# niclasborlin/dbat

Hardware: AMD Instinct MI355X
Metric: LM iterations/sec (higher is better)
Workload: dtype f64

## Files before the change

### dbat_amd/_hip.py

```python
from __future__ import annotations

import ctypes as C
import os
import sys

import numpy as np

_HERE = os.path.dirname(os.path.abspath(__file__))
LIB_PATH = os.path.join(_HERE, 'libdbat_hip.so')
if os.environ.get('DBAT_AMD_LIB') == 'prof':
    LIB_PATH = os.path.join(_HERE, 'libdbat_hip_prof.so')
elif os.environ.get('DBAT_AMD_LIB', '').endswith('.so'):
    LIB_PATH = os.environ['DBAT_AMD_LIB']
if LIB_PATH != os.path.join(_HERE, 'libdbat_hip.so'):
    sys.stderr.write('[dbat_amd] DBAT_AMD_LIB: loading %s instead of the product library\n' % LIB_PATH)

ABI_VERSION = 5
DAMP = {'none': 0, 'gm': 0, 'gna': 1, 'lm': 2, 'lmp': 3}

OK, EINVAL, EUNSUPPORTED, EDEVICE, ENOMEM = 0, -101, -102, -103, -104


class DbatHipUnavailable(RuntimeError):
    pass
# ... 138 lines not shown
    'dbat_hip_ray_angles': (C.c_int, [_H, _dp, _dp, _dp, _ip, _ip]),
    'dbat_hip_debug_ray_angles_host': (C.c_int, [C.POINTER(Problem), _dp, _dp]),
    'dbat_hip_default_robust_options': (C.c_int, [C.c_int32, C.POINTER(RobustOptions)]),
    'dbat_hip_robust_weights': (C.c_int, [_H, _dp, C.POINTER(RobustOptions), _dp, _dp, _dp]),
    'dbat_hip_set_obs_weights': (C.c_int, [_H, _dp]),
    'dbat_hip_solve_robust': (C.c_int, [_H, C.POINTER(Options), C.POINTER(RobustOptions), _dp, C.POINTER(Result),
                                        _dp, _dp, _dp, _dp, C.POINTER(RobustResult), _dp]),
}
DEBUG_SYMBOLS = {
    'dbat_hip_debug_plan_digest': (C.c_int, [C.POINTER(Problem), C.POINTER(C.c_uint64), C.c_int32, C.c_char_p, C.c_int32]),
    'dbat_hip_debug_heavy_plan_selftest': (C.c_int, [C.POINTER(Problem), _dp]),
    'dbat_hip_debug_batch_stats': (C.c_int, [C.POINTER(Problem), C.POINTER(C.c_int64)]),
    'dbat_hip_debug_model_eval_host': (C.c_int, [C.c_int32, C.c_int32, C.c_int32, _dp, _dp, C.c_double,
                                                 _dp, _dp, _dp, _dp, _dp, _dp]),
    'dbat_hip_debug_ray_angles_ms': (C.c_int, [_H, _dp, C.POINTER(C.c_int64)]),
}

_lib = None


def load():
    global _lib
    if _lib is not None:
        return _lib
    if not os.path.exists(LIB_PATH):
        raise DbatHipUnavailable(
            '%s not built: run `python -c "import __graft_entry__ as g; g.build()"` or '
            '`make -C dbat_amd/csrc` (needs hipcc).  There is no CPU fallback.' % LIB_PATH)
    try:
        try:
# ... 407 lines not shown
    def set_x(self, x):
        x = np.ascontiguousarray(x, float)
        check(self.lib.dbat_hip_set_x(self.h, dptr(x)))

    def bench_step(self, lam=0.0, scale=False):
        ms = np.zeros(16)
        check(self.lib.dbat_hip_bench_step(self.h, float(lam), int(bool(scale)), dptr(ms)))
        return ms

    def chol_stats(self):
        a = (C.c_int64 * 6)()
        check(self.lib.dbat_hip_chol_stats(self.h, a))
        keys = ('order_padded', 'tile_tasks', 'tile_products', 'tile_rows', 'nested_dissection', 'dataflow')
        return dict(zip(keys, [int(v) for v in a]))

    def info(self):
        a = (C.c_int64 * 24)()
        check(self.lib.dbat_hip_info(self.h, a))
        keys = ('NS', 'n_batches', 'max_k', 'n_obs_shard', 'n_pts_shard', 'BT', 'ncolmax', 'n_tiles',
                'domain_sharding', 'reduced_doubles_per_factorisation', 'vector_doubles_per_linearisation',
                'n_top_cams', 'factor_tile_rows', 'tasks_domain', 'tasks_top', 'tile_kernel_mfma',
                'heavy_tasks', 'heavy_mfma', 'heavy_row_groups', 'heavy_scratch_bytes', 'heavy_points', 'heavy_obs',
                'heavy_ksteps_per_task', 'heavy_algorithmic_flops')
        return dict(zip(keys, [int(v) for v in a]))


def structure_key(s, device=0, shard_rank=0, shard_count=1, _problem=None):
    prob, keep = _problem if _problem is not None else problem_from_struct(s, device, shard_rank, shard_count)
    k = (C.c_uint64 * 2)()
    check(load().dbat_hip_structure_key(C.byref(prob), k))
# ... 178 lines not shown
```

### dbat_amd/csrc/dbat_core.hip

```cpp
#include <hip/hip_runtime.h>
#include <rocblas/rocblas.h>
#include <rocsolver/rocsolver.h>
#include <rccl/rccl.h>

#include <chrono>
#include <cmath>
#include <cstdio>
#include <cstdlib>
#include <memory>
#include <string>
#include <thread>
#include <type_traits>
#include <utility>
#include <atomic>
#include <vector>

#include "../../include/dbat_hip.h"
#include "chol_df.hpp"
#include "kernels.hpp"
#include "sig.hpp"
#include "heavy.hpp"
#include "plan.hpp"
#include "resect.hpp"
#include "robust.hpp"
// ... 104 lines not shown
    enum class TileRoute { none, sig, tile3, tile2 } route = TileRoute::none;
    DevBuf<int64_t> o_row, batch_start, x2z, giant_start, cm_chunk_start;
    DevBuf<int32_t> cm_pt, cm_chunk_cam, tile_order;
    DevBuf<double> cm_uv, cm_w;
    int64_t n_cm_chunks = 0, n_cm_chunks_all = 0;
    DevBuf<double> giant_W;
    int64_t ngiant = 0;
    bool use_heavy = false;
    HeavyDev hv{};
    DevBuf<int32_t> hv_obs_dst, hv_pt_io0, hv_io_dst, hv_io_pt, hv_pt_y, hv_grp_nb, hv_grp_row, hv_task, hv_ops;
    DevBuf<uint8_t> hv_obs_ld, hv_obs_ioloc, hv_io_ld;
    DevBuf<double> hv_Z;
    int giant_threads = 256;
    DevBuf<CamRec> cams, cams_f;
    bool cams_at_lin = false;

    const char *env_df_trace = nullptr;
    DevBuf<unsigned> gctr;
    DevBuf<double> gpart, rpart;
    DevBuf<double> z, zt, dz, zlin, vtmp, vtmp2, xbuf;
    DevBuf<double> red;
    DevBuf<double> jn2c, dscale, rhs, Vinv, gp, jn2p, partial, scal;
    DevBuf<int> info;
    DevBuf<double> linv, ldiag;
    DataflowChol dfchol;
    DataflowChol dfchol_ip;
    bool use_perm = true;
    bool mg_subtree = false;
    DevBuf<uint8_t> piv_have;
    bool chol_in_place = false;
// ... 205 lines not shown
        lds_cov = ((size_t)P.BT * P.ncolmax * 3 + (size_t)P.BT * 6) * sizeof(double);
        tile2_pc = TILE2_PC;
        static_assert(Plan::PMAX == 256 / 2, "k_build_tile2 / k_build_tile3 lay out NPROD / 2 points per batch");
        lds_tile2 = ((size_t)TILE2_NBUF * 3 * tile2_pc * TILE_LD + (size_t)2 * Plan::PMAX * 9 + (size_t)Plan::PMAX * 15 + TILE_LD) * sizeof(double);
        lds_tile3 = ((size_t)TILE3_NBUF * 3 * TILE3_PC * TILE_LD + (size_t)2 * Plan::PMAX * 9 + (size_t)2 * Plan::PMAX * 9 + TILE_LD) * sizeof(double);
        use_tile2 = P.BT == 256 && P.ncolmax <= 15;
        if (ntiles <= 0) route = TileRoute::none;
        else if (use_sig) route = TileRoute::sig;
        else if (use_tile2 && !P.with_io && tile_ncx == 6) route = TileRoute::tile3;
        else if (use_tile2 && (tile_ncx == 14 || tile_ncx == 15)) route = TileRoute::tile2;
        else throw DeviceError{"internal: tiles without a tile kernel"};
        partial.alloc((size_t)4 * std::max<int64_t>(std::max<int64_t>(std::max<int64_t>(nb + ntiles + ngiant + (int64_t)P.sg_chunk.size() / 8, n_cm_chunks_all), 2048), 1));
        HIPCHK(hipMemcpy(z.p, P.z0.data(), P.NZ * 8, hipMemcpyHostToDevice));
        HIPCHK(hipMemset(dz.p, 0, P.NZ * 8));
        HIPCHK(hipMemset(zt.p, 0, P.NZ * 8));
        precompute_image_side();
        HIPCHK(hipDeviceSynchronize());
        lapi("work arrays, image side");
    }

    void precompute_image_side() {
        uv_pre = !P.with_io;
        d.o_uv_raw = o_uv.p; d.uv_pre = uv_pre ? 1 : 0;
        if (!uv_pre || nobs == 0) return;
        prep_cams(z.p, cams_f.p);
        if (!o_rhs.p) o_rhs.alloc((size_t)2 * nobs);
        with_value<2, 3, 4, 5>(P.model, [&](auto M) {
            launch<k_uv_to_rhs<M>>(dim3((unsigned)cdiv(nobs, 256)), dim3(256), 0, d.nK, d.nP, cams_f.p, nobs, o_cam.p, o_uv.p, o_rhs.p);
            if (n_cm_chunks_all > 0) launch<k_uv_to_rhs_cm<M>>(dim3((unsigned)n_cm_chunks_all), dim3(256), 0, d.nK, d.nP, cams_f.p, cm_chunk_cam.p, cm_chunk_start.p, cm_uv.p);
            if (use_sig && sg_nchunks > 0) launch<k_uv_to_rhs_sig<M>>(dim3((unsigned)sg_nchunks), dim3(64), 0, d.nK, d.nP, cams_f.p, sg_chunk.p, sg_gcam.p, sg_uv.p);
// ... 6 lines not shown
        HIPCHK(hipMemcpyAsync(z.p, P.z0.data(), P.NZ * 8, hipMemcpyHostToDevice, stream));
        HIPCHK(hipMemcpyAsync(io_fixed.p, P.io_fixed.data(), P.io_fixed.size() * 8, hipMemcpyHostToDevice, stream));
        if (d.any_prior) {
            HIPCHK(hipMemcpyAsync(z_prw.p, P.z_prw.data(), P.NZ * 8, hipMemcpyHostToDevice, stream));
            HIPCHK(hipMemcpyAsync(z_prv.p, P.z_prv.data(), P.NZ * 8, hipMemcpyHostToDevice, stream));
        }
        HIPCHK(hipStreamSynchronize(stream));
        if (uv_pre && io_changed && nobs > 0) {
            HIPCHK(hipMemcpy(cm_uv.p, P.cm_uv.data(), P.cm_uv.size() * 8, hipMemcpyHostToDevice));
            if (use_sig && sg_nchunks > 0) HIPCHK(hipMemcpy(sg_uv.p, P.sg_uv.data(), P.sg_uv.size() * 8, hipMemcpyHostToDevice));
            d.o_uv = o_uv.p;
            precompute_image_side();
            HIPCHK(hipStreamSynchronize(stream));
        }
        cams_at_lin = false; have_lin = false; s_valid = false; pend_build = false; lin_pending = false;
        lambda_lin = 0; scale_lin = 0; f_lin = 0; trace_jtj = 0; near_singular = false; chol_in_place = false; replicate_next = false;
        n_res_evals = n_lin = n_solves = n_trace_only = 0;
    }

    static int env_grid_obs() { return std::min(std::max(1, env_int("DBAT_HIP_GRID_OBS", 1536)), 1 << 20); }

    int64_t tile_kernel_mfma() const {
        if (route == TileRoute::none) return 0;
        int64_t n = 0;
        if (route == TileRoute::sig) {
            for (int64_t t = 0; t < ntiles; ++t) {
                const int nio = tile_ncx > 6 ? P.tile_io_start[t + 1] - P.tile_io_start[t] : 0;
                for (int64_t q = P.sg_tile_chunk0[t]; q < P.sg_tile_chunk0[t + 1]; ++q) {
                    const int npts = P.sg_chunk[8 * q + 1], k = P.sg_chunk[8 * q + 2];
                    const int ppr = std::min(SIG_PPR, 64 / std::max(k, 1)), rbk = (6 * k + nio + 1 + 15) >> 4;
// ... 92 lines not shown
        do_allreduce(zgather.p, P.NZ);
        return zgather.p;
    }
    void read_scal(double *host, int n) {
        if (n <= 32) {
            HIPCHK(hipMemcpyAsync(hpin, scal.p, n * sizeof(double), hipMemcpyDeviceToHost, stream));
            sync();
            memcpy(host, hpin, n * sizeof(double));
            return;
        }
        HIPCHK(hipMemcpyAsync(host, scal.p, n * sizeof(double), hipMemcpyDeviceToHost, stream));
        sync();
    }
    void prep_cams(const double *zz, CamRec *into = nullptr) {
        if (!into) { into = cams.p; cams_at_lin = false; }
        launch<k_cam_prep>(dim3((unsigned)cdiv(P.nc, 64)), dim3(64), 0, d, zz, into);
    }
    void x_to_z(const double *x_host, double *z_dev) {
        HIPCHK(hipMemcpyAsync(z_dev, P.z0.data(), P.NZ * 8, hipMemcpyHostToDevice, stream));
        if (P.n) {
            HIPCHK(hipMemcpyAsync(xbuf.p, x_host, P.n * 8, hipMemcpyHostToDevice, stream));
            launch<k_scatter_x>(dim3((unsigned)cdiv(P.n, 256)), dim3(256), 0, P.n, x2z.p, xbuf.p, z_dev);
        }
    }
    void z_to_x(const double *z_dev, double *x_host) {
        if (!P.n) return;
        stage(4);
        z_dev = gathered(z_dev);
        launch<k_gather_x>(dim3((unsigned)cdiv(P.n, 256)), dim3(256), 0, P.n, x2z.p, z_dev, xbuf.p);
        HIPCHK(hipMemcpyAsync(x_host, xbuf.p, P.n * 8, hipMemcpyDeviceToHost, stream));
        sync();
    }

// ... 25 lines not shown
        if (!P.n || nt <= 0) return std::max(nt, 0);
        HIPCHK(hipMemcpyAsync(host, trace_dev.p, (size_t)P.n * nt * 8, hipMemcpyDeviceToHost, stream));
        HIPCHK(hipStreamSynchronize(stream));
        for (int k = 0; k < nt; ++k)
            if (!trace_have[k]) std::fill(host + (size_t)P.n * k, host + (size_t)P.n * (k + 1), NAN);
        if ((size_t)P.n * trace_cap * 8 > ((size_t)256 << 20)) {
            DevBuf<double> old;
            std::swap(old.p, trace_dev.p);
            trace_cap = 0;
        }
        return nt;
    }

    double eval_f_step(const double *x, double alpha, const double *pdir, double *out) {
        stage(3);
        if ((int64_t)cdiv(P.NZ, 256) < P.nc) { axpby(1.0, x, alpha, pdir, out); return eval_f(out, nullptr, nullptr); }
        launch<k_axpby_cams>(dim3((unsigned)cdiv(P.NZ, 256)), dim3(256), 0, d, 1.0, x, alpha, pdir, out, cams_f.p);
        return eval_f(out, nullptr, nullptr, true);
    }
    double eval_f(const double *zz, double *r_w_out, double *r_unw_out, bool cams_ready = false) {
        stage(3);
        if (!cams_ready) prep_cams(zz, cams_f.p);
        mark(6);
        const bool res_tail = n_cm_chunks_all > 0 && n_cm_chunks_all <= 512 && !d.any_prior && !multi() && !r_w_out && !r_unw_out;
        with_value<2, 3, 4, 5>(P.model, [&](auto M) {
            with_value<false, true>(uv_pre, [&](auto PRE) {
                if (n_cm_chunks_all > 0)
                    launch<k_residual_cm<M, PRE>>(dim3((unsigned)n_cm_chunks_all), dim3(256), 0, d, zz, cams_f.p, cm_pt.p, cm_uv.p, pw ? cm_w.p : (const double *)nullptr,
                                                  cm_chunk_cam.p, cm_chunk_start.p, partial.p, res_tail ? gctr.p + 1 : (unsigned *)nullptr, scal.p, hpin, res_tail ? ++mb_seq : 0ull);
                mark(7);
                if (r_w_out || r_unw_out) launch<k_residual<M, PRE>>(dim3(grid_obs), dim3(256), 0, d, zz, cams_f.p, rpart.p, r_w_out, r_unw_out);
            });
        });
// ... 167 lines not shown
            for (int i = 0; i < 8; ++i) fprintf(stderr, " %s=%.2f", nm[i], h[i] * 0.01 / (double)std::max<int64_t>(ntiles, 1));
            fprintf(stderr, "\n");
            memset(h, 0, sizeof(h));
            HIPCHK(hipMemcpyToSymbol(HIP_SYMBOL(g_tile2_prof), h, sizeof(h)));
        } else if ((d.ablate & 32) && use_tile2) {
            unsigned long long h[16];
            HIPCHK(hipStreamSynchronize(stream));
            HIPCHK(hipMemcpyFromSymbol(h, HIP_SYMBOL(g_tile2_prof), sizeof(h)));
            static const char *nm[12] = {"stage(wait freed)", "P1", "pbarrier", "P2", "P3", "drain", "cons wait full", "cons zero+free", "tail/flush", "loop head", "cons product", "cons wait done"};
            fprintf(stderr, "[tile2 prof, us per tile avg over %d tiles]", (int)ntiles);
            for (int i = 0; i < 12; ++i) fprintf(stderr, " %s=%.2f", nm[i], h[i] * 0.01 / (double)std::max<int64_t>(ntiles, 1));
            fprintf(stderr, "\n");
            memset(h, 0, sizeof(h));
            HIPCHK(hipMemcpyToSymbol(HIP_SYMBOL(g_tile2_prof), h, sizeof(h)));
        }
        launch<k_build_tail>(dim3(grid_zs), dim3(1024), 0, d, zz, partial.p, npart, jn2p.p, gpart.p, gctr.p + 2, red_scal,
                zz != zlin.p ? zlin.p : (double *)nullptr);
    }
    bool pend_build = false;
    double pend_lambda = 0;
    int pend_scale = 0;
    void request_build(double lambda, int scale) {
        pend_build = true; pend_lambda = lambda; pend_scale = scale;
        lambda_lin = lambda; scale_lin = scale;
    }
    void ensure_build() {
        if (!pend_build) return;
        build(z.p, pend_lambda, pend_scale, true);
    }
    void settle_lin_point() {
        if (!pend_build) return;
        copy(zlin.p, z.p);
        cams_at_lin = false; s_valid = false; have_lin = true;
    }
    void allreduce_vectors() {
        if (!multi()) return;
        do_allreduce(g_c, 2 * P.NS + 8);
    }
    void trace_only_pass(const double *zz) {
        stage(0);
        prep_cams(zz);
        if (n_cm_chunks_all > 0) {
            with_value<2, 3, 4, 5>(P.model, [&](auto M) { with_value<6, 14, 15, MAXCOL>(tile_ncx, [&](auto NCX) {
                launch<k_trace_cm<M, NCX>>(dim3((unsigned)n_cm_chunks_all), dim3(256), 0, d, zz, cams.p, cm_pt.p, cm_uv.p, pw ? cm_w.p : (const double *)nullptr,
                                           cm_chunk_cam.p, cm_chunk_start.p, partial.p);
            }); });
        }
// ... 37 lines not shown
        launch<k_finish>(dim3((unsigned)cdiv(P.NS, 256)), dim3(256), 0, d, zz, lambda, scale, S, g_c, g_red, diagU, jn2c.p, dscale.p,
                gpart.p, gctr.p + 3, (const double *)red_scal, scal.p, hpin, mg_subtree && multi() ? (const uint8_t *)z_mine.p : (const uint8_t *)nullptr,
                ride ? info.p : (int *)nullptr, ride ? df_ctl : (int *)nullptr, ride ? df_q : (unsigned long long *)nullptr, ride ? df_nq : 0);
        if (ride) dfchol.reset_done = true;
        if (scale)
            launch<k_envelope_op>(dim3((unsigned)P.NS), dim3(256), 0, S, ldS, (int)P.NS, env_tail0, col_bend.p, (const double *)dscale.p, (double *)nullptr,
                                  (unsigned long long *)nullptr);
    }

    int factor_solve_enqueue() {
        if (mg_subtree && !multi())
            throw UsageError{"this handle is one of several shards: attach a communicator (dbat_hip_comm_init) or an all-reduce "
                             "callback (dbat_hip_set_allreduce) before linearising or solving"};
        stage(1);
        mark(2);
        if (use_perm && !chol_in_place && mg_subtree && multi()) {
            dfchol.solve_domain(stream, S, ldS, linv.p, info.p, ldiag.p);
            mark(8);
            do_allreduce(dfchol.top_tiles(), dfchol.top_tiles_count());
            mark(9);
            dfchol.solve_top(stream, ldS, rhs.p, linv.p, info.p, ldiag.p, dscale.p, dz.p);
        } else if (use_perm && !chol_in_place) dfchol.solve(stream, S, ldS, rhs.p, linv.p, info.p, ldiag.p, dscale.p, dz.p);
        else dfchol_ip.solve(stream, S, ldS, rhs.p, linv.p, info.p, ldiag.p, dscale.p, dz.p);
        HIPCHK(hipGetLastError());
        if (env_df_trace) (use_perm && !chol_in_place ? dfchol : dfchol_ip).dump_trace(stream, env_df_trace);
        mark(3);
        ++n_solves;
        return 0;
    }
    void backsub_enqueue() {
        stage(2);
        mark(4);
        const bool sig_bs = use_sig && P.sg_backsub_ok;
        const int64_t b_first = sig_bs ? P.nb_tiled : 0;
        const int64_t n_sig_wg = sig_bs ? cdiv(sg_nchunks, 4) : 0;
        if (n_sig_wg > 0) {
            with_value<2, 3, 4, 5>(P.model, [&](auto M) { with_value<6, 14>(tile_ncx, [&](auto NCX) {
                launch<k_backsub_sig<M, NCX>>(dim3((unsigned)n_sig_wg), dim3(256), 0, d, zlin.p, cams.p, Vinv.p, gp.p, dz.p, partial.p + 2 * (nb + ngiant), sg_chunk.p,
                                              (int)sg_nchunks, sg_gcam.p, sg_uv.p, pw ? sg_w.p : (const double *)nullptr);
            }); });
        }
        if (nb > b_first) {
            with_value<2, 3, 4, 5>(P.model, [&](auto M) { with_value<6, 14, 15, MAXCOL>(tile_ncx, [&](auto NCX) {
                launch<k_backsub<M, NCX>>(dim3((unsigned)(nb - b_first)), dim3(P.BT), lds_back, d, zlin.p, cams.p, Vinv.p, gp.p, dz.p, partial.p, (int)b_first);
            }); });
        }
        if (ngiant > 0) {
            with_value<2, 3, 4, 5>(P.model, [&](auto M) { with_value<false, true>(P.with_io, [&](auto IO) {
                launch<k_backsub_giant<M, IO>>(dim3((unsigned)ngiant), dim3(giant_threads), 0, d, zlin.p, cams.p, Vinv.p, gp.p, dz.p, partial.p + 2 * nb);
            }); });
        }
        mark(5);
        launch<k_prior_jv>(dim3(grid_zs), dim3(1024), 0, d, zlin.p, dz.p, g_c, gp.p, gpart.p, gctr.p + 4,
                (const double *)(partial.p + 2 * b_first), nb - b_first + ngiant + n_sig_wg, (const double *)ldiag.p, pivmm.p,
                (const int *)info.p, scal.p, multi() ? (double *)nullptr : hpin, ++mb_seq,
                mg_subtree && multi() ? (const uint8_t *)piv_have.p : (const uint8_t *)nullptr);
    }
    bool near_singular = false;
    const bool pivot_stats = env_on("DBAT_HIP_PIVOT_STATS");
    double rcond_est = 0.0;
    int chol_info = 0;
    double piv_last[4] = {0, 0, 0, 0};
    bool solve(double &JpJp, double &rJp, double &pp) {
        ensure_build();
        if (!s_valid) build(zlin.p, lambda_lin, scale_lin);
        s_valid = false;
        factor_solve_enqueue();
// ... 391 lines not shown
                                         (const double *)o_w_base.p, o_w.p, (const int32_t *)(use_sig ? sg_map.p : nullptr), sg_w.p,
                                         (const int32_t *)cm_map.p, cm_w.p);
        s_valid = false;
    }
    void robust_omega_ip(double *host) {
        if (!robust_on) { std::fill(host, host + P.no, 1.0); return; }
        DevBuf<double> t;
        t.alloc((size_t)std::max<int64_t>(P.no, 1));
        HIPCHK(hipMemsetAsync(t.p, 0, (size_t)P.no * sizeof(double), stream));
        if (nobs > 0) launch<k_scatter_rows1>(dim3(robust_grid()), dim3(256), 0, nobs, (const int64_t *)o_row.p, (const double *)omega.p, t.p);
        if (multi()) do_allreduce(t.p, P.no);
        HIPCHK(hipMemcpyAsync(host, t.p, (size_t)P.no * sizeof(double), hipMemcpyDeviceToHost, stream));
        HIPCHK(hipStreamSynchronize(stream));
    }
    void jtimes(const double *v, double &JvJv, double &rJv, double &vv) {
        if (!cams_at_lin) { prep_cams(zlin.p); cams_at_lin = true; }
        with_value<2, 3, 4, 5>(P.model, [&](auto M) { with_value<6, 14, 15, MAXCOL>(tile_ncx, [&](auto NCX) {
            launch<k_jtimes<M, NCX>>(dim3(grid_obs), dim3(256), 0, d, zlin.p, cams.p, v, partial.p);
        }); });
        launch<k_prior_jv>(dim3(grid_zs), dim3(1024), 0, d, zlin.p, v, g_c, gp.p, gpart.p, gctr.p + 4,
                (const double *)partial.p, (int64_t)grid_obs, (const double *)nullptr, pivmm.p, (const int *)info.p, scal.p, (double *)nullptr, 0ull, (const uint8_t *)nullptr);
        do_allreduce(scal.p, 8);
        double h[8];
        read_scal(h, 8);
        JvJv = h[0] + h[4]; rJv = h[1] + h[5]; vv = h[6];
    }
    double dot_owned(const double *a, const double *b) {
        launch<k_dot>(dim3(grid_z), dim3(256), 0, P.NZ, z_mine.p, a, b, partial.p);
        launch<k_sum_partials<1>>(dim3(1), dim3(1024), 0, partial.p, (int64_t)grid_z, scal.p, 0);
        do_allreduce(scal.p, 1);
        double s;
        read_scal(&s, 1);
        return s;
    }
    void axpby(double a, const double *x, double b, const double *y2, double *y) {
        launch<k_axpby>(dim3((unsigned)cdiv(P.NZ, 256)), dim3(256), 0, P.NZ, a, x, b, y2, y);
    }
    void gradient(double *g) {
        launch<k_gradient>(dim3((unsigned)cdiv(P.NZ, 256)), dim3(256), 0, d, g_c, gp.p, g);
    }
    void colnorm2(double *out) {
        launch<k_jn2>(dim3((unsigned)cdiv(P.NZ, 256)), dim3(256), 0, d, jn2c.p, jn2p.p, out);
    }
    void jac_blocks(const double *zz, double *a, double *b, double *cc) {
        with_value<2, 3, 4, 5>(P.model, [&](auto M) { launch<k_jac_blocks<M>>(dim3((unsigned)cdiv(nobs, 256)), dim3(256), 0, d, zz, cams.p, a, b, cc); });
    }
    void copy(double *dst, const double *src) { HIPCHK(hipMemcpyAsync(dst, src, P.NZ * 8, hipMemcpyDeviceToDevice, stream)); }
    void accept_trial() { std::swap(z.p, zt.p); }
};


struct LoopOut {
    std::vector<double> res, damp, aux;
    int code = 0, iters = 0;
    double f_final = 0;
};

static void export_residuals(Core &c, const double *zdev, double *r_unw, double *r_wgt, double *f);
static void jtimes_rows(Core &c, const double *v_dev, double *Jv);

static void keep_Jp(Core &c, const dbat_hip_options &o, const double *p_dev, std::vector<double> &Jp) {
    if (!o.term_fun) return;
    Jp.resize((size_t)c.P.m);
// ... 1219 lines not shown
    if (!h || !st) { g_err = "null argument"; return DBAT_HIP_EINVAL; }
    const Core &c = *h->core;
    const DataflowChol &f = c.use_perm ? c.dfchol : c.dfchol_ip;
    st[0] = f.n; st[1] = f.ntasks; st[2] = f.n_products; st[3] = f.nT; st[4] = c.use_perm ? 1 : 0; st[5] = 1;
    return DBAT_HIP_OK;
}

int dbat_hip_build_kernel_name(const dbat_hip_handle *h, char *buf, int32_t buf_len) {
    if (!h || !buf || buf_len < 2) { g_err = "null argument"; return DBAT_HIP_EINVAL; }
    const Core &c = *h->core;
    using R = Core::TileRoute;
    const char *nm = c.route == R::sig ? "k_build_sig" : c.route == R::tile3 ? "k_build_tile3" : c.route == R::tile2 ? "k_build_tile2"
                   : c.use_heavy ? "k_heavy_z + k_heavy_syrk" : "k_build";
    snprintf(buf, (size_t)buf_len, "%s", nm);
    return DBAT_HIP_OK;
}

int dbat_hip_info(const dbat_hip_handle *h, int64_t *info) {
    if (!h || !info) { g_err = "null argument"; return DBAT_HIP_EINVAL; }
    const Core &c = *h->core;
    info[0] = c.P.NS; info[1] = c.nb; info[2] = c.P.max_k; info[3] = c.nobs;
    info[4] = c.P.pt_hi - c.P.pt_lo; info[5] = c.P.BT; info[6] = c.P.ncolmax; info[7] = c.ntiles;
    info[8] = c.mg_subtree ? 1 : 0;
    info[9] = c.mg_subtree ? c.dfchol.top_tiles_count() : (c.P.nranks > 1 ? c.pk_s_count : 0);
    info[10] = c.P.nranks > 1 ? (c.mg_subtree ? 2 * c.P.NS + 8 : 3 * c.P.NS + 8) : 0;
    info[11] = c.mg_subtree ? c.P.nd.n_top_cams : 0;
    info[12] = c.use_perm ? c.dfchol.nT : 0;
    info[13] = c.mg_subtree ? c.dfchol.ntasks : 0; info[14] = c.mg_subtree ? c.dfchol.ntasksB : 0;
    info[15] = c.tile_kernel_mfma();
    for (int i = 16; i < 24; ++i) info[i] = 0;
// ... 187 lines not shown
```

### dbat_amd/csrc/env.hpp

```cpp
#pragma once
#include <cstdlib>
#include <cstring>
#include <string>

extern char **environ;

namespace dbat {

#ifdef DBAT_HIP_PROFILING
constexpr bool kProfilingBuild = true;
#else
constexpr bool kProfilingBuild = false;
#endif

struct EnvSwitch { const char *name; bool measurement; const char *what; const char *values = nullptr; };
static const EnvSwitch kEnvSwitches[] = {
    {"DBAT_HIP_SIG", false, "0: signature kernels off, 2: on wherever a chunk's rows fit (default: by group length)", "0|1|2"},
    {"DBAT_HIP_SIG_IOS_OFF", false, "self-calibration: IO rows by LDS atomics in every tile"},
    {"DBAT_HIP_CMAX", false, "cameras per tile (0: column-list kernel only)"},
    {"DBAT_HIP_BT", false, "observations per batch (128 | 256)", "128|256"},
    {"DBAT_HIP_TILE_BMIN", false, "fewest batches a tile may be capped at (default 2)"},
    {"DBAT_HIP_HEAVY", false, "0: heavy / giant points by the column-list kernels (pair terms by global atomics) instead of the matrix-core path", "0|1"},
    {"DBAT_HIP_HEAVY_KS", false, "heavy / giant points: k-steps per task of k_heavy_syrk at most (default: by the amount of work, 12 ... 96)"},
    {"DBAT_HIP_GIANT_THREADS", false, "threads of the giant-point kernels (64 | 128 | 256)", "64|128|256"},
// ... 1 lines not shown
    {"DBAT_HIP_ND_OFF", false, "no nested dissection"},
    {"DBAT_HIP_ND_LEAF", false, "leaf size of the dissection"},
    {"DBAT_HIP_ND_PAD_ALL", false, "every block of the dissection on a tile boundary"},
    {"DBAT_HIP_ND_JOIN_SMALL", false, "separators up to that many rows join their child's last tile"},
    {"DBAT_HIP_DF_SPLIT", false, "factorisation: helper tasks for sums longer than this many products (default 96)"},
    {"DBAT_HIP_DF_CHUNK", false, "factorisation: products per helper task (default 32)"},
    {"DBAT_HIP_DF_CHAIN", false, "factorisation: 0 = diagonal tiles as ordinary tasks (no chain role), 1 = chain role whatever the pattern", "0|1"},
    {"DBAT_HIP_DF_CHAIN_WG", false, "factorisation: workgroups of the chain role at most (default 32)"},
    {"DBAT_HIP_DF_L2", false, "factorisation: 1 = finished tiles of the compact layout are read through the L2", "0|1"},
    {"DBAT_HIP_COV_DENSE", false, "posterior covariance: the dense inverse of the reduced system (rocsolver_dpotri) instead of the selected inversion"},
    {"DBAT_HIP_SPRANK_OFF", false, "structural rank from the counting conditions only"},
    {"DBAT_HIP_PLAN_THREADS", false, "threads of the host plan (default: hardware concurrency, at most 32)"},
    {"DBAT_HIP_PLAN_GRAIN", false, "elements per thread below which a pass of the host plan is not split (tests: 1)"},
    {"DBAT_HIP_PLAN_STATS", false, "1: print layout statistics, 2: also the wall time of every section of the plan"},
    {"DBAT_HIP_PIVOT_STATS", false, "print the pivot extremes and the rcond estimate of every solve"},
    {"DBAT_HIP_ABLATE", true, "k_build_sig / tile kernels: switch phases off (results are wrong), phase clocks"},
    {"DBAT_HIP_DF_TRACE", true, "per-task clocks of the factorisation, written to this file"},
    {"DBAT_HIP_DF_TRACE_POTF2", true, "with DF_TRACE: clocks inside the chain role's factorisations as well"},
    {"DBAT_HIP_DF_ABLATE", true, "factorisation: operand tiles of the products not fetched (1: L(i,j), 2: both, 3: and no flag looks) -- timing only, wrong results", "0|1|2|3"},
    {"DBAT_HIP_DF_ORDER", true, "one of the candidate task orders instead of the simulated best"},
    {"DBAT_HIP_DF_GRID", true, "workgroups of the factorisation"},
    {"DBAT_HIP_GRID_OBS", true, "launch size of the observation-parallel kernels"},
};

inline const char *env_get(const char *name) {
    for (const EnvSwitch &e : kEnvSwitches)
        if (!strcmp(e.name, name)) return (e.measurement && !kProfilingBuild) ? nullptr : getenv(name);
    return nullptr;
}
inline int env_int(const char *name, int dflt) { const char *e = env_get(name); return e ? atoi(e) : dflt; }
// ... 27 lines not shown
```

### dbat_amd/csrc/kernels.hpp

```cpp
#pragma once
#include <hip/hip_runtime.h>

#include "model.hpp"

namespace dbat {

struct DevProblem {
    int nc, np, nIOrows, nK, nP, nIOu, ncolmax, BT;
    int64_t NS, NZ, nobs, nb;
    int64_t ldS;
    const int32_t *cam_ncol, *cam_col, *cam_iorow;
    const uint32_t *cam_eo_est;
    const int32_t *io_src;
    const double *io_fixed;
    const double *px;
    const double *cam_w;
    const uint8_t *z_est, *z_mine;
    const double *z_prw, *z_prv;
    const int32_t *o_cam, *o_pt;
    const double *o_uv;
    const double *o_uv_raw;
    int uv_pre;
    const double *o_w;
    const uint32_t *o_seg;
// ... 2729 lines not shown
        out[0] = acc[3]; out[1] = acc[4]; out[4] = acc[0]; out[5] = acc[1]; out[6] = acc[2];
        out[7] = info && __hip_atomic_load(info, __ATOMIC_RELAXED, __HIP_MEMORY_SCOPE_AGENT) != 0 ? 1.0 : 0.0;
        out[2] = 0.0; out[3] = 0.0;
        if (mailbox) {
            mailbox[0] = acc[3]; mailbox[1] = acc[4]; mailbox[4] = acc[0]; mailbox[5] = acc[1]; mailbox[6] = acc[2];
            for (int q = 0; q < 4; ++q)
                mailbox[40 + q] = __longlong_as_double((long long)__hip_atomic_load(pivmm + q, __ATOMIC_RELAXED, __HIP_MEMORY_SCOPE_AGENT));
            const int hi = __hip_atomic_load(info, __ATOMIC_RELAXED, __HIP_MEMORY_SCOPE_AGENT);
            long long w = hi;
            mailbox[44] = __longlong_as_double(w);
            mailbox_done(mailbox, seq);
        }
    }
}

__global__ __launch_bounds__(256) void k_dot(int64_t n, const uint8_t *__restrict__ mine,
                                             const double *__restrict__ a, const double *__restrict__ b ,
                                             double *__restrict__ partial) {
    __shared__ double sh[8];
    double acc[1] = {0};
    const int64_t stride = (int64_t)gridDim.x * blockDim.x;
    for (int64_t i = (int64_t)blockIdx.x * blockDim.x + threadIdx.x; i < n; i += stride)
        if (!mine || mine[i]) acc[0] += a[i] * (b ? b[i] : 1.0);
    block_sum<1>(acc, sh);
    if (threadIdx.x == 0) partial[blockIdx.x] = acc[0];
}

__global__ void k_axpby(int64_t n, double a, const double *__restrict__ x, double b,
                        const double *__restrict__ y2, double *__restrict__ y) {
    const int64_t i = (int64_t)blockIdx.x * blockDim.x + threadIdx.x;
// ... 87 lines not shown
```

### dbat_amd/csrc/sig.hpp

```cpp
#pragma once
#include <cstddef>
#include <type_traits>

#include "kernels.hpp"

namespace dbat {

constexpr int SIG_LDK = 18;
constexpr int SIG_PPR = 6;
constexpr int SIG_KMAXR = 13;
constexpr int SIG_NW = 8;
constexpr int SIG_CAMW = (int)(offsetof(CamRec, ncol) / 8) + 1;
constexpr int SIG_CAMW_IO = (int)((sizeof(CamRec) + 7) / 8);
constexpr int SIG_STILE = 8064;
#ifndef DBAT_SIG_IO_WAVES
#define DBAT_SIG_IO_WAVES 4
#endif
constexpr int SIG_IO_CAMS = DBAT_SIG_IO_WAVES == 8 ? 16 : 21;
__host__ __device__ constexpr int sig_stile(bool io) { return io && DBAT_SIG_IO_WAVES == 8 ? 6336 : SIG_STILE; }
__host__ __device__ constexpr int sig_cams(bool io) { return io ? SIG_IO_CAMS : 21; }

struct SigLds {
    int next_chunk, abort_;
    int flush_turn;
// ... 662 lines not shown
        else if (NCX > 6 && ios == 2)
            build_sig_tile<MODEL, RB, NCX, (NCX > 6 ? 2 : 0), PW>(d, tile, (int)ti, z, cams, lambda, scale, S, g_red, Vinv, gp, jn2p, partial, pivmm, sg_chunk, sg_tile_chunk0, sg_lc, sg_uv, sg_w, tile_ctr + 2, sy, sh);
        else
            build_sig_tile<MODEL, RB, NCX, 0, PW>(d, tile, (int)ti, z, cams, lambda, scale, S, g_red, Vinv, gp, jn2p, partial, pivmm, sg_chunk, sg_tile_chunk0, sg_lc, sg_uv, sg_w, tile_ctr + 2, sy, sh);
        __syncthreads();
    }
}

template <int MODEL, int NCX>
__global__ __launch_bounds__(256) void k_backsub_sig(DevProblem d, const double *__restrict__ z,
                                                     const CamRec *__restrict__ cams,
                                                     const double *__restrict__ Vinv, const double *__restrict__ gp,
                                                     double *__restrict__ dz, double *__restrict__ partial ,
                                                     const int32_t *__restrict__ sg_chunk, int nchunks,
                                                     const int32_t *__restrict__ sg_gcam,
                                                     const double *__restrict__ sg_uv, const double *__restrict__ sg_w) {
    constexpr int CW = (int)((sizeof(CamRec) + 7) / 8);
    __shared__ double sh[8];
    __shared__ double crec[4][SIG_KMAXR][CW];
    __shared__ double dcs[4][SIG_KMAXR][NCX];
    const int t = threadIdx.x, lane = t & 63;
    const int wv = t >> 6;
    const int ch = __builtin_amdgcn_readfirstlane(blockIdx.x * 4 + (t >> 6));
    double acc[2] = {0, 0};
    if (ch < nchunks) {
        const int32_t *cd = sg_chunk + 8 * (int64_t)ch;
        const int pt0 = cd[0], npts = cd[1], k = cd[2], gm = cd[4], gi0 = cd[5], uv0 = cd[6];
        const int mycam = lane < k ? sg_gcam[16 * (int64_t)ch + lane] : 0;
        for (int base = 0; base < k * CW; base += 64) {
            const int idx = base + lane, c = min(idx / CW, k - 1), f = idx - c * CW;
            const int cam = __builtin_amdgcn_ds_bpermute(4 * c, mycam);
            if (idx < k * CW) crec[wv][c][f] = reinterpret_cast<const double *>(cams + cam)[f];
        }
        __builtin_amdgcn_wave_barrier();
        for (int idx = lane; idx < k * NCX; idx += 64) {
            const int c = idx / NCX, a = idx - c * NCX;
            const CamRec &C = *reinterpret_cast<const CamRec *>(crec[wv][c]);
            const bool on = a < (NCX > 6 ? min(C.ncol, NCX) : 6) && (NCX > 6 || ((C.eo_est >> a) & 1u));
            dcs[wv][c][a] = on ? dz[C.col[a]] : 0.0;
        }
        __builtin_amdgcn_wave_barrier();
        const int G = npts > 32 ? 64 : (npts > 16 ? 32 : (npts > 8 ? 16 : 8));
        const int pi = lane & (G - 1), jh = lane / G, jstep = 64 / G;
        const bool act = pi < npts;
        const int pt = pt0 + (act ? pi : 0);
        const int64_t zp = d.NS + 3 * (int64_t)pt;
        const double Q[3] = {z[zp], z[zp + 1], z[zp + 2]};
        const unsigned est = (d.z_est[zp] ? 1u : 0u) | (d.z_est[zp + 1] ? 2u : 0u) | (d.z_est[zp + 2] ? 4u : 0u);
        const double2 *uvp = reinterpret_cast<const double2 *>(sg_uv), *wp = reinterpret_cast<const double2 *>(sg_w);
        const int64_t q0 = uv0 + gi0 + (act ? pi : 0);
        double sB[3] = {0, 0, 0}, V0[6] = {0, 0, 0, 0, 0, 0}, tt2 = 0;
        auto sweep = [&](auto per_obs_w) {
        for (int j = jh; j < k; j += jstep) {
            const CamRec &C = *reinterpret_cast<const CamRec *>(crec[wv][j]);
            double2 uv = {0, 0};
            if constexpr (NCX > 6) uv = uvp[q0 + (int64_t)j * gm];
            double w0, w1;
            if constexpr (decltype(per_obs_w)::value) { const double2 ww = wp[q0 + (int64_t)j * gm]; w0 = ww.x; w1 = ww.y; }
            else { w0 = C.w[0]; w1 = C.w[1]; }
            double B[2][3], t0 = 0, t1 = 0;
            if constexpr (NCX > 6) {
                obs_step_dot<MODEL, true>(C, Q, uv.x, uv.y, w0, w1, est, dcs[wv][j], t0, t1, B);
            } else {
                sig_step_dot6(C, Q, w0, w1, dcs[wv][j], t0, t1, B);
            }
#define DBAT_ACC2(acc, a, b, c, e) acc = __builtin_fma(a, b, __builtin_fma(c, e, acc))
            DBAT_ACC2(tt2, t0, t0, t1, t1);
            DBAT_ACC2(sB[0], B[0][0], t0, B[1][0], t1);
            DBAT_ACC2(sB[1], B[0][1], t0, B[1][1], t1);
            DBAT_ACC2(sB[2], B[0][2], t0, B[1][2], t1);
            DBAT_ACC2(V0[0], B[0][0], B[0][0], B[1][0], B[1][0]);
            DBAT_ACC2(V0[1], B[0][0], B[0][1], B[1][0], B[1][1]);
            DBAT_ACC2(V0[2], B[0][0], B[0][2], B[1][0], B[1][2]);
            DBAT_ACC2(V0[3], B[0][1], B[0][1], B[1][1], B[1][1]);
            DBAT_ACC2(V0[4], B[0][1], B[0][2], B[1][1], B[1][2]);
            DBAT_ACC2(V0[5], B[0][2], B[0][2], B[1][2], B[1][2]);
#undef DBAT_ACC2
        }
        };
        if (sg_w) sweep(std::true_type{}); else sweep(std::false_type{});
        for (int m = G; m < 64; m <<= 1) {
#pragma unroll
            for (int c = 0; c < 3; ++c) sB[c] += lane_get(sB[c], lane ^ m);
#pragma unroll
            for (int c = 0; c < 6; ++c) V0[c] += lane_get(V0[c], lane ^ m);
            tt2 += lane_get(tt2, lane ^ m);
        }
        {
            const double s0 = gp[3 * (int64_t)pt] + sB[0], s1 = gp[3 * (int64_t)pt + 1] + sB[1], s2 = gp[3 * (int64_t)pt + 2] + sB[2];
            double p0, p1, p2;
            point_block_solve_neg(Vinv + 6 * (int64_t)pt, s0, s1, s2, p0, p1, p2);
            const double d0 = (est & 1u) ? p0 : 0.0, d1 = (est & 2u) ? p1 : 0.0, d2 = (est & 4u) ? p2 : 0.0;
            if (act && lane == pi) {
                dz[zp] = d0; dz[zp + 1] = d1; dz[zp + 2] = d2;
                acc[0] = tt2 + 2.0 * (d0 * sB[0] + d1 * sB[1] + d2 * sB[2])
                       + d0 * (V0[0] * d0 + V0[1] * d1 + V0[2] * d2) + d1 * (V0[1] * d0 + V0[3] * d1 + V0[4] * d2)
                       + d2 * (V0[2] * d0 + V0[4] * d1 + V0[5] * d2);
            }
        }
    }
    block_sum<2>(acc, sh);
    if (t == 0) { partial[2 * blockIdx.x] = acc[0]; partial[2 * blockIdx.x + 1] = acc[1]; }
}

}
```

Measured before the change: 629.2.

## Fuse trial-point formation and point dot products into signature back-substitution tail

On the single-rank signature back-substitution route, the back-substitution kernel now writes the trial point z+dz for point unknowns and accumulates g'p and p'p per point. A new k_prior_jv_cams kernel covers only the camera unknowns, forms zt and the trial camera records, and reduces the combined partials. The following eval_f_step then skips its own axpby/cam-prep pass when a dirty-tracking flag shows the trial is still valid. It also hoists the per-point gp/Vinv loads and prefetches per-observation weights in the 6-column kernel. The cost is extra validity state that must be invalidated on every write, plus a debug entry point.

```diff
diff --git a/dbat_amd/_hip.py b/dbat_amd/_hip.py
--- a/dbat_amd/_hip.py
+++ b/dbat_amd/_hip.py
@@ -176,6 +176,7 @@
     'dbat_hip_debug_model_eval_host': (C.c_int, [C.c_int32, C.c_int32, C.c_int32, _dp, _dp, C.c_double,
                                                  _dp, _dp, _dp, _dp, _dp, _dp]),
     'dbat_hip_debug_ray_angles_ms': (C.c_int, [_H, _dp, C.POINTER(C.c_int64)]),
+    'dbat_hip_debug_backsub_tail': (C.c_int, [_H, C.POINTER(C.c_int64), C.POINTER(C.c_double), _dp, _dp, _dp]),
 }
 
 _lib = None
@@ -613,6 +614,18 @@
         keys = ('order_padded', 'tile_tasks', 'tile_products', 'tile_rows', 'nested_dissection', 'dataflow')
         return dict(zip(keys, [int(v) for v in a]))
 
+    def backsub_tail(self, vectors=False):
+        a = (C.c_int64 * 8)()
+        f = C.c_double(0)
+        check(self.lib.dbat_hip_debug_backsub_tail(self.h, a, C.byref(f), None, None, None))
+        out = dict(zip(('route', 'solves', 'reused', 'formed', 'ready', 'NZ', 'NS'), [int(v) for v in a]))
+        out['f_trial'] = f.value
+        if vectors:
+            v = [np.empty(out['NZ']) for _ in range(3)]
+            check(self.lib.dbat_hip_debug_backsub_tail(self.h, a, C.byref(f), dptr(v[0]), dptr(v[1]), dptr(v[2])))
+            out.update(zlin=v[0], dz=v[1], zt=v[2])
+        return out
+
     def info(self):
         a = (C.c_int64 * 24)()
         check(self.lib.dbat_hip_info(self.h, a))
diff --git a/dbat_amd/csrc/dbat_core.hip b/dbat_amd/csrc/dbat_core.hip
--- a/dbat_amd/csrc/dbat_core.hip
+++ b/dbat_amd/csrc/dbat_core.hip
@@ -142,6 +142,16 @@
     int giant_threads = 256;
     DevBuf<CamRec> cams, cams_f;
     bool cams_at_lin = false;
+    const bool bs_tail_env = env_int("DBAT_HIP_BACKSUB_TAIL", 1) != 0;
+    bool bs_tail_ok = false;
+    bool z_at_lin = false, trial_ready = false;
+    double f_trial_last = NAN;
+    int64_t n_bs_tail = 0, n_trial_reused = 0, n_trial_formed = 0;
+    bool bs_tail_route() const { return bs_tail_ok && !multi(); }
+    void wrote(const void *p) {
+        if (p == (const void *)z.p || p == (const void *)zlin.p) { z_at_lin = false; trial_ready = false; }
+        else if (p == (const void *)dz.p || p == (const void *)zt.p || p == (const void *)cams_f.p) trial_ready = false;
+    }
 
     const char *env_df_trace = nullptr;
     DevBuf<unsigned> gctr;
@@ -377,6 +387,12 @@
         HIPCHK(hipMemcpy(z.p, P.z0.data(), P.NZ * 8, hipMemcpyHostToDevice));
         HIPCHK(hipMemset(dz.p, 0, P.NZ * 8));
         HIPCHK(hipMemset(zt.p, 0, P.NZ * 8));
+        {
+            int64_t sg_pts = 0;
+            for (size_t q = 0; q + 8 <= P.sg_chunk.size(); q += 8) sg_pts += P.sg_chunk[q + 1];
+            bs_tail_ok = bs_tail_env && P.nranks == 1 && !mg_subtree && use_sig && P.sg_backsub_ok && sg_nchunks > 0 &&
+                         nb == P.nb_tiled && ngiant == 0 && sg_pts == P.np && P.NZ == P.NS + 3 * (int64_t)P.np;
+        }
         precompute_image_side();
         HIPCHK(hipDeviceSynchronize());
         lapi("work arrays, image side");
@@ -413,6 +429,7 @@
             HIPCHK(hipStreamSynchronize(stream));
         }
         cams_at_lin = false; have_lin = false; s_valid = false; pend_build = false; lin_pending = false;
+        z_at_lin = false; trial_ready = false;
         lambda_lin = 0; scale_lin = 0; f_lin = 0; trace_jtj = 0; near_singular = false; chol_in_place = false; replicate_next = false;
         n_res_evals = n_lin = n_solves = n_trace_only = 0;
     }
@@ -535,9 +552,11 @@
     }
     void prep_cams(const double *zz, CamRec *into = nullptr) {
         if (!into) { into = cams.p; cams_at_lin = false; }
+        wrote(into);
         launch<k_cam_prep>(dim3((unsigned)cdiv(P.nc, 64)), dim3(64), 0, d, zz, into);
     }
     void x_to_z(const double *x_host, double *z_dev) {
+        wrote(z_dev);
         HIPCHK(hipMemcpyAsync(z_dev, P.z0.data(), P.NZ * 8, hipMemcpyHostToDevice, stream));
         if (P.n) {
             HIPCHK(hipMemcpyAsync(xbuf.p, x_host, P.n * 8, hipMemcpyHostToDevice, stream));
@@ -593,9 +612,15 @@
 
     double eval_f_step(const double *x, double alpha, const double *pdir, double *out) {
         stage(3);
-        if ((int64_t)cdiv(P.NZ, 256) < P.nc) { axpby(1.0, x, alpha, pdir, out); return eval_f(out, nullptr, nullptr); }
+        if (trial_ready && z_at_lin && alpha == 1.0 && x == z.p && pdir == dz.p && out == zt.p && bs_tail_route()) {
+            ++n_trial_reused;
+            return f_trial_last = eval_f(out, nullptr, nullptr, true);
+        }
+        ++n_trial_formed;
+        if ((int64_t)cdiv(P.NZ, 256) < P.nc) { axpby(1.0, x, alpha, pdir, out); return f_trial_last = eval_f(out, nullptr, nullptr); }
+        wrote(out); wrote(cams_f.p);
         launch<k_axpby_cams>(dim3((unsigned)cdiv(P.NZ, 256)), dim3(256), 0, d, 1.0, x, alpha, pdir, out, cams_f.p);
-        return eval_f(out, nullptr, nullptr, true);
+        return f_trial_last = eval_f(out, nullptr, nullptr, true);
     }
     double eval_f(const double *zz, double *r_w_out, double *r_unw_out, bool cams_ready = false) {
         stage(3);
@@ -793,6 +818,8 @@
             memset(h, 0, sizeof(h));
             HIPCHK(hipMemcpyToSymbol(HIP_SYMBOL(g_tile2_prof), h, sizeof(h)));
         }
+        trial_ready = false;
+        z_at_lin = zz == z.p || (zz == zlin.p && z_at_lin);
         launch<k_build_tail>(dim3(grid_zs), dim3(1024), 0, d, zz, partial.p, npart, jn2p.p, gpart.p, gctr.p + 2, red_scal,
                 zz != zlin.p ? zlin.p : (double *)nullptr);
     }
@@ -810,6 +837,7 @@
     void settle_lin_point() {
         if (!pend_build) return;
         copy(zlin.p, z.p);
+        z_at_lin = true;
         cams_at_lin = false; s_valid = false; have_lin = true;
     }
     void allreduce_vectors() {
@@ -877,6 +905,7 @@
                              "callback (dbat_hip_set_allreduce) before linearising or solving"};
         stage(1);
         mark(2);
+        trial_ready = false;
         if (use_perm && !chol_in_place && mg_subtree && multi()) {
             dfchol.solve_domain(stream, S, ldS, linv.p, info.p, ldiag.p);
             mark(8);
@@ -897,10 +926,13 @@
         const bool sig_bs = use_sig && P.sg_backsub_ok;
         const int64_t b_first = sig_bs ? P.nb_tiled : 0;
         const int64_t n_sig_wg = sig_bs ? cdiv(sg_nchunks, 4) : 0;
+        const bool tail = bs_tail_route() && sig_bs && n_sig_wg > 0;
+        trial_ready = false;
         if (n_sig_wg > 0) {
             with_value<2, 3, 4, 5>(P.model, [&](auto M) { with_value<6, 14>(tile_ncx, [&](auto NCX) {
                 launch<k_backsub_sig<M, NCX>>(dim3((unsigned)n_sig_wg), dim3(256), 0, d, zlin.p, cams.p, Vinv.p, gp.p, dz.p, partial.p + 2 * (nb + ngiant), sg_chunk.p,
-                                              (int)sg_nchunks, sg_gcam.p, sg_uv.p, pw ? sg_w.p : (const double *)nullptr);
+                                              (int)sg_nchunks, sg_gcam.p, sg_uv.p, pw ? sg_w.p : (const double *)nullptr,
+                                              tail ? zt.p : (double *)nullptr, tail ? 4 : 2);
             }); });
         }
         if (nb > b_first) {
@@ -914,6 +946,16 @@
             }); });
         }
         mark(5);
+        if (tail) {
+            const int64_t need = std::max<int64_t>(cdiv(P.NS, 1024), cdiv((int64_t)P.nc, 16));
+            const unsigned grid = (unsigned)(d.any_prior ? grid_zs : std::max<int64_t>(1, std::min<int64_t>(need, grid_zs)));
+            launch<k_prior_jv_cams>(dim3(grid), dim3(1024), 0, d, zlin.p, dz.p, g_c, gpart.p, gctr.p + 4,
+                    (const double *)(partial.p + 2 * (nb + ngiant)), n_sig_wg, (const double *)ldiag.p, pivmm.p,
+                    (const int *)info.p, scal.p, hpin, ++mb_seq, zt.p, cams_f.p);
+            trial_ready = true;
+            ++n_bs_tail;
+            return;
+        }
         launch<k_prior_jv>(dim3(grid_zs), dim3(1024), 0, d, zlin.p, dz.p, g_c, gp.p, gpart.p, gctr.p + 4,
                 (const double *)(partial.p + 2 * b_first), nb - b_first + ngiant + n_sig_wg, (const double *)ldiag.p, pivmm.p,
                 (const int *)info.p, scal.p, multi() ? (double *)nullptr : hpin, ++mb_seq,
@@ -1335,6 +1377,7 @@
         HIPCHK(hipStreamSynchronize(stream));
     }
     void jtimes(const double *v, double &JvJv, double &rJv, double &vv) {
+        trial_ready = false;
         if (!cams_at_lin) { prep_cams(zlin.p); cams_at_lin = true; }
         with_value<2, 3, 4, 5>(P.model, [&](auto M) { with_value<6, 14, 15, MAXCOL>(tile_ncx, [&](auto NCX) {
             launch<k_jtimes<M, NCX>>(dim3(grid_obs), dim3(256), 0, d, zlin.p, cams.p, v, partial.p);
@@ -1355,19 +1398,22 @@
         return s;
     }
     void axpby(double a, const double *x, double b, const double *y2, double *y) {
+        wrote(y);
         launch<k_axpby>(dim3((unsigned)cdiv(P.NZ, 256)), dim3(256), 0, P.NZ, a, x, b, y2, y);
     }
     void gradient(double *g) {
+        wrote(g);
         launch<k_gradient>(dim3((unsigned)cdiv(P.NZ, 256)), dim3(256), 0, d, g_c, gp.p, g);
     }
     void colnorm2(double *out) {
+        wrote(out);
         launch<k_jn2>(dim3((unsigned)cdiv(P.NZ, 256)), dim3(256), 0, d, jn2c.p, jn2p.p, out);
     }
     void jac_blocks(const double *zz, double *a, double *b, double *cc) {
         with_value<2, 3, 4, 5>(P.model, [&](auto M) { launch<k_jac_blocks<M>>(dim3((unsigned)cdiv(nobs, 256)), dim3(256), 0, d, zz, cams.p, a, b, cc); });
     }
-    void copy(double *dst, const double *src) { HIPCHK(hipMemcpyAsync(dst, src, P.NZ * 8, hipMemcpyDeviceToDevice, stream)); }
-    void accept_trial() { std::swap(z.p, zt.p); }
+    void copy(double *dst, const double *src) { wrote(dst); HIPCHK(hipMemcpyAsync(dst, src, P.NZ * 8, hipMemcpyDeviceToDevice, stream)); }
+    void accept_trial() { std::swap(z.p, zt.p); z_at_lin = false; trial_ready = false; }
 };
 
 
@@ -2617,6 +2663,22 @@
                    : c.use_heavy ? "k_heavy_z + k_heavy_syrk" : "k_build";
     snprintf(buf, (size_t)buf_len, "%s", nm);
     return DBAT_HIP_OK;
+}
+
+int dbat_hip_debug_backsub_tail(dbat_hip_handle *h, int64_t *out, double *f_trial, double *zlin, double *dz, double *zt) {
+    API_TRY
+    if (!h || !out) { g_err = "null argument"; return DBAT_HIP_EINVAL; }
+    Core &c = *h->core;
+    DeviceGuard dev_guard(c.device);
+    out[0] = c.bs_tail_route() ? 1 : 0; out[1] = c.n_bs_tail; out[2] = c.n_trial_reused; out[3] = c.n_trial_formed;
+    out[4] = c.trial_ready ? 1 : 0; out[5] = c.P.NZ; out[6] = c.P.NS; out[7] = 0;
+    if (f_trial) *f_trial = c.f_trial_last;
+    c.sync();
+    const std::pair<double *, const double *> cp[3] = {{zlin, c.zlin.p}, {dz, c.dz.p}, {zt, c.zt.p}};
+    for (const auto &q : cp)
+        if (q.first) HIPCHK(hipMemcpy(q.first, q.second, (size_t)c.P.NZ * 8, hipMemcpyDeviceToHost));
+    return DBAT_HIP_OK;
+    API_CATCH
 }
 
 int dbat_hip_info(const dbat_hip_handle *h, int64_t *info) {
diff --git a/dbat_amd/csrc/env.hpp b/dbat_amd/csrc/env.hpp
--- a/dbat_amd/csrc/env.hpp
+++ b/dbat_amd/csrc/env.hpp
@@ -39,6 +39,7 @@
     {"DBAT_HIP_PLAN_GRAIN", false, "elements per thread below which a pass of the host plan is not split (tests: 1)"},
     {"DBAT_HIP_PLAN_STATS", false, "1: print layout statistics, 2: also the wall time of every section of the plan"},
     {"DBAT_HIP_PIVOT_STATS", false, "print the pivot extremes and the rcond estimate of every solve"},
+    {"DBAT_HIP_BACKSUB_TAIL", false, "0: g'p, p'p and the trial point z + p by their own passes behind the back-substitution (k_prior_jv over every unknown, k_axpby_cams) instead of inside it (default 1)", "0|1"},
     {"DBAT_HIP_ABLATE", true, "k_build_sig / tile kernels: switch phases off (results are wrong), phase clocks"},
     {"DBAT_HIP_DF_TRACE", true, "per-task clocks of the factorisation, written to this file"},
     {"DBAT_HIP_DF_TRACE_POTF2", true, "with DF_TRACE: clocks inside the chain role's factorisations as well"},
diff --git a/dbat_amd/csrc/kernels.hpp b/dbat_amd/csrc/kernels.hpp
--- a/dbat_amd/csrc/kernels.hpp
+++ b/dbat_amd/csrc/kernels.hpp
@@ -2767,6 +2767,66 @@
     }
 }
 
+__global__ __launch_bounds__(1024) void k_prior_jv_cams(DevProblem d, const double *__restrict__ z,
+                                                       const double *__restrict__ v, const double *__restrict__ g_c,
+                                                       double *__restrict__ partial, unsigned *__restrict__ ctr,
+                                                       const double *__restrict__ bs_partial, int64_t nbs,
+                                                       const double *__restrict__ ldiag, unsigned long long *__restrict__ pivmm,
+                                                       const int *__restrict__ info, double *__restrict__ out,
+                                                       double *__restrict__ mailbox, unsigned long long seq,
+                                                       double *__restrict__ zt, CamRec *__restrict__ cams_t) {
+    __shared__ double sh[80];
+    double acc[5] = {0, 0, 0, 0, 0};
+    const int64_t stride = (int64_t)gridDim.x * blockDim.x, gid = (int64_t)blockIdx.x * blockDim.x + threadIdx.x;
+    double pmin = 1e300, pmax = 0.0;
+    for (int64_t i = gid; i < d.NS; i += stride) {
+        if (ldiag && d.z_est[i]) {
+            double p = ldiag[i];
+            p = p == p ? p : 0.0;
+            pmin = fmin(pmin, p); pmax = fmax(pmax, p);
+        }
+        const double vr = v[i];
+        zt[i] = z[i] + vr;
+        const double w = d.any_prior ? d.z_prw[i] : 0.0, vi = d.z_est[i] ? vr : 0.0;
+        if (w > 0) acc[0] += w * vi * vi;
+        acc[3] += g_c[i] * vi;
+        acc[4] += vi * vi;
+    }
+    if (d.any_prior)
+        for (int64_t i = d.NS + gid; i < d.NZ; i += stride) {
+            const double w = d.z_prw[i];
+            if (w > 0 && d.z_est[i]) { const double vi = v[i]; acc[0] += w * vi * vi; }
+        }
+    if ((threadIdx.x & 63) == 0)
+        for (int64_t c = gid >> 6; c < d.nc; c += stride >> 6)
+            cam_prep_one(d, [=](int64_t q) { return z[q] + v[q]; }, (int)c, cams_t);
+    if (ldiag && (int64_t)blockIdx.x * blockDim.x < d.NS) {
+        for (int off = 32; off > 0; off >>= 1) {
+            pmin = fmin(pmin, __shfl_down(pmin, off, 64));
+            pmax = fmax(pmax, __shfl_down(pmax, off, 64));
+        }
+        if ((threadIdx.x & 63) == 0 && pmax > 0.0) {
+            atomicMin(pivmm + 2, (unsigned long long)__double_as_longlong(fmax(pmin, 0.0)));
+            atomicMax(pivmm + 3, (unsigned long long)__double_as_longlong(pmax));
+        }
+        __builtin_amdgcn_s_waitcnt(0);
+    }
+    if (grid_sum<5, 4, 1>(acc, sh, partial, ctr, bs_partial, nbs, 4) && threadIdx.x == 0) {
+        out[0] = acc[1]; out[1] = acc[2]; out[4] = acc[0]; out[5] = acc[3]; out[6] = acc[4];
+        out[7] = info && __hip_atomic_load(info, __ATOMIC_RELAXED, __HIP_MEMORY_SCOPE_AGENT) != 0 ? 1.0 : 0.0;
+        out[2] = 0.0; out[3] = 0.0;
+        if (mailbox) {
+            mailbox[0] = acc[1]; mailbox[1] = acc[2]; mailbox[4] = acc[0]; mailbox[5] = acc[3]; mailbox[6] = acc[4];
+            for (int q = 0; q < 4; ++q)
+                mailbox[40 + q] = __longlong_as_double((long long)__hip_atomic_load(pivmm + q, __ATOMIC_RELAXED, __HIP_MEMORY_SCOPE_AGENT));
+            const int hi = __hip_atomic_load(info, __ATOMIC_RELAXED, __HIP_MEMORY_SCOPE_AGENT);
+            long long w = hi;
+            mailbox[44] = __longlong_as_double(w);
+            mailbox_done(mailbox, seq);
+        }
+    }
+}
+
 __global__ __launch_bounds__(256) void k_dot(int64_t n, const uint8_t *__restrict__ mine,
                                              const double *__restrict__ a, const double *__restrict__ b ,
                                              double *__restrict__ partial) {
diff --git a/dbat_amd/csrc/sig.hpp b/dbat_amd/csrc/sig.hpp
--- a/dbat_amd/csrc/sig.hpp
+++ b/dbat_amd/csrc/sig.hpp
@@ -700,32 +700,21 @@
                                                      double *__restrict__ dz, double *__restrict__ partial ,
                                                      const int32_t *__restrict__ sg_chunk, int nchunks,
                                                      const int32_t *__restrict__ sg_gcam,
-                                                     const double *__restrict__ sg_uv, const double *__restrict__ sg_w) {
+                                                     const double *__restrict__ sg_uv, const double *__restrict__ sg_w,
+                                                     double *__restrict__ zt, int pstride) {
     constexpr int CW = (int)((sizeof(CamRec) + 7) / 8);
-    __shared__ double sh[8];
+    constexpr bool HOIST = NCX <= 6;
+    __shared__ double sh[16];
     __shared__ double crec[4][SIG_KMAXR][CW];
     __shared__ double dcs[4][SIG_KMAXR][NCX];
     const int t = threadIdx.x, lane = t & 63;
     const int wv = t >> 6;
     const int ch = __builtin_amdgcn_readfirstlane(blockIdx.x * 4 + (t >> 6));
-    double acc[2] = {0, 0};
+    double acc[4] = {0, 0, 0, 0};
     if (ch < nchunks) {
         const int32_t *cd = sg_chunk + 8 * (int64_t)ch;
         const int pt0 = cd[0], npts = cd[1], k = cd[2], gm = cd[4], gi0 = cd[5], uv0 = cd[6];
         const int mycam = lane < k ? sg_gcam[16 * (int64_t)ch + lane] : 0;
-        for (int base = 0; base < k * CW; base += 64) {
-            const int idx = base + lane, c = min(idx / CW, k - 1), f = idx - c * CW;
-            const int cam = __builtin_amdgcn_ds_bpermute(4 * c, mycam);
-            if (idx < k * CW) crec[wv][c][f] = reinterpret_cast<const double *>(cams + cam)[f];
-        }
-        __builtin_amdgcn_wave_barrier();
-        for (int idx = lane; idx < k * NCX; idx += 64) {
-            const int c = idx / NCX, a = idx - c * NCX;
-            const CamRec &C = *reinterpret_cast<const CamRec *>(crec[wv][c]);
-            const bool on = a < (NCX > 6 ? min(C.ncol, NCX) : 6) && (NCX > 6 || ((C.eo_est >> a) & 1u));
-            dcs[wv][c][a] = on ? dz[C.col[a]] : 0.0;
-        }
-        __builtin_amdgcn_wave_barrier();
         const int G = npts > 32 ? 64 : (npts > 16 ? 32 : (npts > 8 ? 16 : 8));
         const int pi = lane & (G - 1), jh = lane / G, jstep = 64 / G;
         const bool act = pi < npts;
@@ -733,8 +722,31 @@
         const int64_t zp = d.NS + 3 * (int64_t)pt;
         const double Q[3] = {z[zp], z[zp + 1], z[zp + 2]};
         const unsigned est = (d.z_est[zp] ? 1u : 0u) | (d.z_est[zp + 1] ? 2u : 0u) | (d.z_est[zp + 2] ? 4u : 0u);
+        double gpt[3], R[6];
+        auto load_point = [&]() {
+#pragma unroll
+            for (int c = 0; c < 3; ++c) gpt[c] = gp[3 * (int64_t)pt + c];
+#pragma unroll
+            for (int c = 0; c < 6; ++c) R[c] = Vinv[6 * (int64_t)pt + c];
+        };
+        if constexpr (HOIST) load_point();
         const double2 *uvp = reinterpret_cast<const double2 *>(sg_uv), *wp = reinterpret_cast<const double2 *>(sg_w);
         const int64_t q0 = uv0 + gi0 + (act ? pi : 0);
+        double2 ww_n = {0, 0};
+        if constexpr (HOIST) { if (sg_w && jh < k) ww_n = wp[q0 + (int64_t)jh * gm]; }
+        for (int base = 0; base < k * CW; base += 64) {
+            const int idx = base + lane, c = min(idx / CW, k - 1), f = idx - c * CW;
+            const int cam = __builtin_amdgcn_ds_bpermute(4 * c, mycam);
+            if (idx < k * CW) crec[wv][c][f] = reinterpret_cast<const double *>(cams + cam)[f];
+        }
+        __builtin_amdgcn_wave_barrier();
+        for (int idx = lane; idx < k * NCX; idx += 64) {
+            const int c = idx / NCX, a = idx - c * NCX;
+            const CamRec &C = *reinterpret_cast<const CamRec *>(crec[wv][c]);
+            const bool on = a < (NCX > 6 ? min(C.ncol, NCX) : 6) && (NCX > 6 || ((C.eo_est >> a) & 1u));
+            dcs[wv][c][a] = on ? dz[C.col[a]] : 0.0;
+        }
+        __builtin_amdgcn_wave_barrier();
         double sB[3] = {0, 0, 0}, V0[6] = {0, 0, 0, 0, 0, 0}, tt2 = 0;
         auto sweep = [&](auto per_obs_w) {
         for (int j = jh; j < k; j += jstep) {
@@ -742,8 +754,12 @@
             double2 uv = {0, 0};
             if constexpr (NCX > 6) uv = uvp[q0 + (int64_t)j * gm];
             double w0, w1;
-            if constexpr (decltype(per_obs_w)::value) { const double2 ww = wp[q0 + (int64_t)j * gm]; w0 = ww.x; w1 = ww.y; }
-            else { w0 = C.w[0]; w1 = C.w[1]; }
+            if constexpr (decltype(per_obs_w)::value) {
+                if constexpr (HOIST) {
+                    w0 = ww_n.x; w1 = ww_n.y;
+                    if (j + jstep < k) ww_n = wp[q0 + (int64_t)(j + jstep) * gm];
+                } else { const double2 ww = wp[q0 + (int64_t)j * gm]; w0 = ww.x; w1 = ww.y; }
+            } else { w0 = C.w[0]; w1 = C.w[1]; }
             double B[2][3], t0 = 0, t1 = 0;
             if constexpr (NCX > 6) {
                 obs_step_dot<MODEL, true>(C, Q, uv.x, uv.y, w0, w1, est, dcs[wv][j], t0, t1, B);
@@ -773,20 +789,27 @@
             tt2 += lane_get(tt2, lane ^ m);
         }
         {
-            const double s0 = gp[3 * (int64_t)pt] + sB[0], s1 = gp[3 * (int64_t)pt + 1] + sB[1], s2 = gp[3 * (int64_t)pt + 2] + sB[2];
+            if constexpr (!HOIST) load_point();
+            const double s0 = gpt[0] + sB[0], s1 = gpt[1] + sB[1], s2 = gpt[2] + sB[2];
             double p0, p1, p2;
-            point_block_solve_neg(Vinv + 6 * (int64_t)pt, s0, s1, s2, p0, p1, p2);
+            point_block_solve_neg(R, s0, s1, s2, p0, p1, p2);
             const double d0 = (est & 1u) ? p0 : 0.0, d1 = (est & 2u) ? p1 : 0.0, d2 = (est & 4u) ? p2 : 0.0;
             if (act && lane == pi) {
                 dz[zp] = d0; dz[zp + 1] = d1; dz[zp + 2] = d2;
+                if (zt) { zt[zp] = Q[0] + d0; zt[zp + 1] = Q[1] + d1; zt[zp + 2] = Q[2] + d2; }
                 acc[0] = tt2 + 2.0 * (d0 * sB[0] + d1 * sB[1] + d2 * sB[2])
                        + d0 * (V0[0] * d0 + V0[1] * d1 + V0[2] * d2) + d1 * (V0[1] * d0 + V0[3] * d1 + V0[4] * d2)
                        + d2 * (V0[2] * d0 + V0[4] * d1 + V0[5] * d2);
-            }
-        }
-    }
-    block_sum<2>(acc, sh);
-    if (t == 0) { partial[2 * blockIdx.x] = acc[0]; partial[2 * blockIdx.x + 1] = acc[1]; }
+                acc[2] = gpt[0] * d0 + gpt[1] * d1 + gpt[2] * d2;
+                acc[3] = d0 * d0 + d1 * d1 + d2 * d2;
+            }
+        }
+    }
+    block_sum<4>(acc, sh);
+    if (t == 0) {
+        partial[(int64_t)pstride * blockIdx.x] = acc[0]; partial[(int64_t)pstride * blockIdx.x + 1] = acc[1];
+        if (pstride == 4) { partial[4 * (int64_t)blockIdx.x + 2] = acc[2]; partial[4 * (int64_t)blockIdx.x + 3] = acc[3]; }
+    }
 }
 
 }
```

Result: no change. 628.5 (-0.1%).
